# RazorClient/Stark-prover

Measured on AMD Instinct MI355X. Metric: FRI commit field-elems/sec at codeword 2^24; achieved HBM GB/s vs peak, higher is better.
Workload: dtype u32; 1 GPU; fri_commit codeword 2^24, blowup 8 (d=2^21), SHA-256 Merkle per layer, 21 rounds; codeword_log2=24, per_gpu_log2=24, blowup=8, field=p=3*2^30+1, parallelism=single GPU

## Files before the change

stark-prover_amd/csrc/fri_layer.hip:

```cpp
#include <cassert>
#include "fri_internal.hpp"
#include "sha256_fast.hpp"
#include "sha256_quad.hpp"

namespace fri {

#ifdef FRI_STAMPS
#define STAMP_WITH(on, i, fn)                                  \
    do {                                                       \
        if (on) t.st->stamps[t.k][(i)] = fn();                 \
    } while (0)
#else
#define STAMP_WITH(on, i, fn) do {} while (0)
#endif
#define STAMP(on, i) STAMP_WITH(on, i, __builtin_amdgcn_s_memrealtime)
#define STAMP_CLK(on, i) STAMP_WITH(on, i, __builtin_amdgcn_s_memtime)

#ifndef FRI_CHAIN_PRIO
#define FRI_CHAIN_PRIO 3
#endif
__device__ __forceinline__ void chain_prio() {
    if (FRI_CHAIN_PRIO > 0) __builtin_amdgcn_s_setprio(FRI_CHAIN_PRIO);
}

// ... 9 lines not shown
}
__device__ __forceinline__ void dg_lds_load(const uint4* p, Dg& d) {
    uint4 a = p[0], b = p[1];
    d.w[0] = a.x; d.w[1] = a.y; d.w[2] = a.z; d.w[3] = a.w; d.w[4] = b.x; d.w[5] = b.y; d.w[6] = b.z; d.w[7] = b.w;
}
__device__ __forceinline__ void dg_lds_store(uint4* p, const Dg& d) {
    p[0] = make_uint4(d.w[0], d.w[1], d.w[2], d.w[3]);
    p[1] = make_uint4(d.w[4], d.w[5], d.w[6], d.w[7]);
}
__device__ __forceinline__ void hnode(const Dg& l, const Dg& r, Dg& o) { shaf::node(l.w, r.w, o.w); }
__device__ __forceinline__ void hleaf(uint32_t v, Dg& o) { shaf::leaf(v, o.w); }
__device__ __forceinline__ void cnode(const Dg& l, const Dg& r, Dg& o) { shaf::node_compact(l.w, r.w, o.w); }
__device__ __forceinline__ void cleaf(uint32_t v, Dg& o) { shaf::leaf_compact(v, o.w); }

__device__ __forceinline__ void pair_level(const uint4* A, uint4* B, uint32_t* out, uint32_t tid, uint32_t cnt,
                                           const shaq::Role& R) {
    if (tid >= max(2 * cnt, 64u)) return;
    const uint32_t q = (tid >> 1) & (cnt - 1), half = (tid & 1u) ^ 1u;
    const bool real = tid < 2 * cnt;
    Dg a, b;
    dg_lds_load(A + 4 * q, a);
    dg_lds_load(A + 4 * q + 2, b);
    uint32_t o[4];
    shaq::node(a.w, b.w, o, R);
    if (!real) return;
    const uint4 v = make_uint4(o[0], o[1], o[2], o[3]);
    B[2 * q + half] = v;
    reinterpret_cast<uint4*>(out + 8 * q)[half] = v;
}

#ifndef FRI_SCHED_PRODUCER
#define FRI_SCHED_PRODUCER 1
#endif
struct SchedLds {
    uint32_t wk[32 * 48];
    uint32_t flag;
};
__device__ __forceinline__ void sched_init(SchedLds* sl) {
    if (FRI_SCHED_PRODUCER && threadIdx.x == 0) sl->flag = 0u;
}
__device__ __forceinline__ void pair_level_s(const uint4* A, uint4* B, uint32_t* out, uint32_t tid, uint32_t cnt,
                                             const shaq::Role& R, SchedLds* sl, uint32_t ord) {
    if (!FRI_SCHED_PRODUCER || cnt > 32) {
        pair_level(A, B, out, tid, cnt, R);
        return;
    }
    const uint32_t wv = tid >> 6;
    if (wv > 1) return;
    const uint32_t lane = tid & 63u;
    const uint32_t q = (lane >> 1) & (cnt - 1), half = (lane & 1u) ^ 1u;
    const bool real = lane < 2 * cnt;
    Dg a, b;
    dg_lds_load(A + 4 * q, a);
    dg_lds_load(A + 4 * q + 2, b);
    if (wv == 1) {
        uint32_t w[16];
#pragma unroll
        for (int i = 0; i < 8; i++) { w[i] = a.w[i]; w[8 + i] = b.w[i]; }
        shaq::produce(w, sl->wk + 48 * q, &sl->flag, 3u * ord, real && (lane & 1u) == 0u, lane == 0u, R);
        return;
    }
    uint32_t o[4];
    shaq::node_ext(a.w, b.w, o, R, sl->wk + 48 * q, &sl->flag, 3u * ord);
    if (!real) return;
    const uint4 v = make_uint4(o[0], o[1], o[2], o[3]);
    B[2 * q + half] = v;
    reinterpret_cast<uint4*>(out + 8 * q)[half] = v;
}

__device__ __forceinline__ void lds_barrier() {
    asm volatile("s_waitcnt lgkmcnt(0)\n\ts_barrier" ::: "memory");
}

__device__ __forceinline__ int wave_max_i(int v) {
#pragma unroll
    for (int off = 32; off > 0; off >>= 1) v = max(v, __shfl_xor(v, off));
    return v;
}

struct Mx3 {
    int m0 = -1, m1 = -1, m2 = -1;
    __device__ __forceinline__ void load(const int32_t* p, uint32_t i) { m0 = p[3 * i]; m1 = p[3 * i + 1]; m2 = p[3 * i + 2]; }
    __device__ __forceinline__ void take(const int32_t* p, uint32_t i) {
        m0 = max(m0, p[3 * i]); m1 = max(m1, p[3 * i + 1]); m2 = max(m2, p[3 * i + 2]);
    }
    __device__ __forceinline__ void store(int32_t* p, uint32_t i) const { p[3 * i] = m0; p[3 * i + 1] = m1; p[3 * i + 2] = m2; }
    __device__ __forceinline__ void wave_max() { m0 = wave_max_i(m0); m1 = wave_max_i(m1); m2 = wave_max_i(m2); }
};
__device__ __forceinline__ void mx3_wave_to_red(Mx3 m, int32_t* red, uint32_t tx) {
    m.wave_max();
    if ((tx & 63) == 0) m.store(red, tx >> 6);
}
__device__ __forceinline__ Mx3 mx3_from_red(const int32_t* red, uint32_t nw) {
    Mx3 m;
    for (uint32_t i = 0; i < nw; i++) m.take(red, i);
    return m;
}
struct Degree { int deg; bool noncanon; };
__device__ __forceinline__ Degree degree_of(int k, const Mx3& m) {
    return {k == 0 ? m.m0 : (m.m1 < 0 ? m.m2 : m.m0), k == 0 && m.m1 >= 0};
}

__device__ __forceinline__ void coef_slice(const LayerTask& t, uint32_t w, uint32_t G, int32_t* red, uint32_t t0,
                                           uint32_t nthr) {
    Mx3 m;
// ... 83 lines not shown

template <bool FOLD, bool COMMIT, uint32_t TPB, bool PAIR = false>
__global__ __launch_bounds__(TPB) void k_layer_leaf(LayerTask t) {
    if (gated_off(t)) return;
    __shared__ uint4 lds[3 * TPB];
    __shared__ int32_t red[3 * (TPB / 64)];
    const uint32_t L = t.L;
    const size_t wg = PAIR ? (size_t)blockIdx.x + t.wg_base : (size_t)blockIdx.x;
    const size_t q = wg * TPB + threadIdx.x;
    uint4 v;
    if (FOLD) {
        const size_t half = (size_t)1 << L;
        const uint32_t beta_m = COMMIT ? t.st->beta_mont[t.k - 1] : (PAIR ? pair_beta(t) : t.beta_m);
        uint4 a = reinterpret_cast<const uint4*>(t.prev)[q];
        uint4 b = reinterpret_cast<const uint4*>(PAIR ? t.prev2 : t.prev + half)[q];
        uint4 x = reinterpret_cast<const uint4*>(t.xinv)[q];
        v.x = fold_one(a.x, b.x, x.x, beta_m); v.y = fold_one(a.y, b.y, x.y, beta_m);
        v.z = fold_one(a.z, b.z, x.z, beta_m); v.w = fold_one(a.w, b.w, x.w, beta_m);
        reinterpret_cast<uint4*>(t.values)[q] = v;
    } else {
        v = reinterpret_cast<const uint4*>(t.values)[q];
    }
    uint32_t* tr = t.tree;
    Dg top;
    quad(v, tr + 8 * level_offset(L, 0), tr + 8 * level_offset(L, 1), q, top);
    if (COMMIT) coef_task(t, blockIdx.x, gridDim.x, red);
    lds_two_levels<TPB>(lds, top, tr + 8 * level_offset(L, 2), tr + 8 * level_offset(L, 3),
                        tr + 8 * level_offset(L, 4), wg * TPB);
}

#ifndef WIDE_PAIR_MAX
#define WIDE_PAIR_MAX (1u << 16)
#endif

__host__ __device__ __forceinline__ uint32_t wide_levels(uint32_t L) { return L <= 8 + TOP_LOG ? 8u : 4u; }

template <bool FOLD, bool COMMIT, bool PAIR = false>
__global__ __launch_bounds__(256) void k_layer_leaf_wide(LayerTask t) {
    if (gated_off(t)) return;
    STAMP(COMMIT && blockIdx.x == 0 && threadIdx.x == 0, 60);
    __shared__ uint4 lds[2 * 256 + 2 * 128];
    __shared__ int32_t red[12];
    __shared__ SchedLds sl;
    sched_init(&sl);
    const uint32_t L = t.L;
    const size_t wg = PAIR ? (size_t)blockIdx.x + t.wg_base : (size_t)blockIdx.x;
    const size_t grid = PAIR ? (size_t)t.wg_total : (size_t)gridDim.x;
    const size_t i = wg * 256 + threadIdx.x;
    uint32_t v;
    if (FOLD) {
        const size_t half = (size_t)1 << L;
        const uint32_t beta_m = COMMIT ? t.st->beta_mont[t.k - 1] : (PAIR ? pair_beta(t) : t.beta_m);
        v = fold_one(t.prev[i], PAIR ? t.prev2[i] : t.prev[i + half], t.xinv[i], beta_m);
        t.values[i] = v;
    } else {
        v = t.values[i];
    }
    uint32_t* tr = t.tree;
    Dg d;
    cleaf(v, d);
    dg_store(tr + 8 * i, d);
    uint4* A = lds;
    uint4* B = lds + 2 * 256;
    dg_lds_store(A + 2 * threadIdx.x, d);
    lds_barrier();
    STAMP(COMMIT && blockIdx.x == 0 && threadIdx.x == 0, 61);
    uint32_t cnt = 256;
    const shaq::Role qr = shaq::role_of(threadIdx.x);
    if (grid * 128 < WIDE_PAIR_MAX) chain_prio();
    const uint32_t nlev = wide_levels(L);
#pragma unroll 1
    for (uint32_t j = 1; j <= nlev; j++) {
        cnt >>= 1;
        uint32_t* out = tr + 8 * (level_offset(L, j) + (wg << (8 - j)));
        if ((size_t)cnt * grid < WIDE_PAIR_MAX) {
            pair_level_s(A, B, out, threadIdx.x, cnt, qr, &sl, j);
        } else if (threadIdx.x < cnt) {
            Dg a, b, o;
            dg_lds_load(A + 4 * threadIdx.x, a);
            dg_lds_load(A + 4 * threadIdx.x + 2, b);
            hnode(a, b, o);
            dg_lds_store(B + 2 * threadIdx.x, o);
            dg_store(out + 8 * threadIdx.x, o);
        }
        if (COMMIT && j == 2 && threadIdx.x >= 128) coef_slice(t, blockIdx.x, gridDim.x, red, 128, 128);
        lds_barrier();
        uint4* tmp = A; A = B; B = tmp;
    }
    if (COMMIT && threadIdx.x == 128) coef_combine(t, blockIdx.x, red, 2);
    STAMP(COMMIT && blockIdx.x == 0 && threadIdx.x == 0, 62);
}

__device__ __forceinline__ void reduce_mx(const int32_t* in, int32_t* out, uint32_t w, uint32_t R) {
    if (threadIdx.x >= 64) return;
    Mx3 m;
    if (threadIdx.x < R) m.load(in, R * w + threadIdx.x);
    m.wave_max();
    if (threadIdx.x == 0) m.store(out, w);
}

__global__ __launch_bounds__(512) void k_tree_mid(uint32_t* tree, uint32_t L, uint32_t l, const DevState* st,
                                                  int gate, const int32_t* mx_in, int32_t* mx_out, uint32_t R) {
    if (st && gate >= 0 && !st->active[gate]) return;
    constexpr uint32_t NIN = 1024;
    __shared__ uint4 lds[NIN + NIN / 2];
    __shared__ SchedLds sl;
    sched_init(&sl);
    uint4* A = lds;
    uint4* B = lds + NIN;
    const uint32_t t = threadIdx.x;
    const size_t base = (size_t)blockIdx.x * NIN;
    const uint32_t* in = tree + 8 * level_offset(L, l);
    {
        Dg a, b, o;
        dg_load(in + 8 * (base + 2 * t), a);
        dg_load(in + 8 * (base + 2 * t + 1), b);
        if (mx_in) reduce_mx(mx_in, mx_out, blockIdx.x, R);
        hnode(a, b, o);
        dg_lds_store(A + 2 * t, o);
        dg_store(tree + 8 * (level_offset(L, l + 1) + (base >> 1) + t), o);
    }
    lds_barrier();
    const shaq::Role qr = shaq::role_of(t);
    uint32_t cnt = NIN / 2;
#pragma unroll 1
    for (uint32_t j = 2; j <= 4; j++) {
        cnt >>= 1;
        uint32_t* out = tree + 8 * (level_offset(L, l + j) + (base >> j));
        const bool narrow = (size_t)cnt * gridDim.x < WIDE_PAIR_MAX;
        if (narrow) {
            pair_level_s(A, B, out, t, cnt, qr, &sl, j);
        } else if (t < cnt) {
            Dg a, b, o;
            dg_lds_load(A + 4 * t, a);
            dg_lds_load(A + 4 * t + 2, b);
            hnode(a, b, o);
            dg_lds_store(B + 2 * t, o);
            dg_store(out + 8 * t, o);
        }
        lds_barrier();
        uint4* tmp = A; A = B; B = tmp;
    }
}

__global__ __launch_bounds__(256) void k_tree_mid8(uint32_t* tree, uint32_t L, uint32_t l, const DevState* st,
                                                   int gate, const int32_t* mx_in, int32_t* mx_out, uint32_t R) {
    if (st && gate >= 0 && !st->active[gate]) return;
    chain_prio();
    __shared__ uint4 lds[256 + 128];
    __shared__ SchedLds sl;
    sched_init(&sl);
    uint4* A = lds;
    uint4* B = lds + 256;
    const uint32_t t = threadIdx.x;
    const size_t base = (size_t)blockIdx.x * 256;
    const uint32_t* in = tree + 8 * level_offset(L, l);
    const shaq::Role qr = shaq::role_of(t);
    {
        const uint32_t q = t >> 1, half = (t & 1u) ^ 1u;
        Dg a, b;
        dg_load(in + 8 * (base + 2 * q), a);
        dg_load(in + 8 * (base + 2 * q + 1), b);
        if (mx_in) reduce_mx(mx_in, mx_out, blockIdx.x, R);
        uint32_t o[4];
        shaq::node(a.w, b.w, o, qr);
        const uint4 v = make_uint4(o[0], o[1], o[2], o[3]);
        A[2 * q + half] = v;
        reinterpret_cast<uint4*>(tree + 8 * (level_offset(L, l + 1) + (base >> 1) + q))[half] = v;
    }
    lds_barrier();
    uint32_t cnt = 128;
#pragma unroll 1
    for (uint32_t j = 2; j <= 8; j++) {
        cnt >>= 1;
        pair_level_s(A, B, tree + 8 * (level_offset(L, l + j) + (base >> j)), t, cnt, qr, &sl, j);
        lds_barrier();
        uint4* tmp = A; A = B; B = tmp;
    }
}

__device__ __forceinline__ void ktouch(const void* sym) {
    uint32_t a, b, c, d;
    asm volatile("s_nop 4\n\t"
                 "s_load_dword %0, %4, 0x0\n\ts_load_dword %1, %4, 0x40\n\t"
                 "s_load_dword %2, %4, 0x80\n\ts_load_dword %3, %4, 0xc0\n\t"
                 "s_waitcnt lgkmcnt(0)"
                 : "=&s"(a), "=&s"(b), "=&s"(c), "=&s"(d)
                 : "s"(sym)
                 : "memory");
}
__device__ __forceinline__ void kcache_touch_sha_tables() {
    ktouch(&shaf::KTAB[0]);
    ktouch(&shaf::PAD_KW_C.kw[0]);
    ktouch(&shaf::PAD_KW_1024.kw[0]);
    ktouch(&shaf::PAD_KW_1536.kw[0]);
}

__device__ __forceinline__ uint32_t hexch(uint32_t nib) { return nib < 10u ? 0x30u + nib : 0x57u + nib; }
__device__ __forceinline__ void hex2(uint32_t x, uint32_t& hi, uint32_t& lo) {
    hi = (hexch(x >> 28) << 24) | (hexch((x >> 24) & 15u) << 16) | (hexch((x >> 20) & 15u) << 8) | hexch((x >> 16) & 15u);
    lo = (hexch((x >> 12) & 15u) << 24) | (hexch((x >> 8) & 15u) << 16) | (hexch((x >> 4) & 15u) << 8) | hexch(x & 15u);
}
__device__ __forceinline__ uint32_t hexhex(uint32_t b) {
    const uint32_t x = ((b & 0xF0u) << 12) | (b & 0x0Fu);
    const uint32_t ge = ((x + 0x00060006u) >> 4) & 0x00010001u;
    return 0x33303330u + x + ge * 0x2F7u;
}

enum { CJ_REHASH = 0, CJ_MID = 2, CJ_ROOT = 3, CJ_FINAL = 6, CJ_END_ROUND = 6, CJ_END_FINAL = 8 };

__device__ __forceinline__ void chan_job(int j, uint32_t cs[8], uint32_t X[4], uint32_t has, const uint4* root_lds,
// ... 65 lines not shown
            dg_lds_store(A + 2 * j, d);
        }
    }
}

__device__ __forceinline__ void level_step(const LayerTask& t, bool stamps, uint32_t it, const uint4* A, uint4* B,
                                           uint32_t* out, uint32_t cnt, const shaq::Role& R, SchedLds* sl,
                                           uint32_t ord) {
    const uint32_t tid = threadIdx.x;
    if (cnt <= 128) {
        STAMP_CLK(stamps && it < 18 && tid == 0, 24 + 2 * it);
        pair_level_s(A, B, out, tid, cnt, R, sl, ord);
        STAMP_CLK(stamps && it < 18 && tid == 0, 25 + 2 * it);
        return;
    }
#pragma unroll 1
    for (uint32_t q = tid; q < cnt; q += blockDim.x) {
        Dg a, b, o;
        dg_lds_load(A + 4 * q, a);
        dg_lds_load(A + 4 * q + 2, b);
#ifdef FRI_STAMPS
        if (stamps && it < 18 && q == 0) asm volatile("s_waitcnt lgkmcnt(0)" ::: "memory");
#endif
        STAMP_CLK(stamps && it < 18 && q == 0, 24 + 2 * it);
        cnode(a, b, o);
        STAMP_CLK(stamps && it < 18 && q == 0, 25 + 2 * it);
        dg_lds_store(B + 2 * q, o);
        dg_store(out + 8 * q, o);
    }
}

__device__ __forceinline__ int chan_drain(const LayerTask& t, int job, int job_end, bool level, uint32_t cnt,
                                           uint32_t cs[8], uint32_t X[4], uint32_t has, const uint4* root_lds,
                                           uint32_t fv, const shaq::Role& R) {
    if (job >= job_end || (level && !(cnt <= 192 && job < CJ_ROOT))) return job;
    do {
        STAMP(threadIdx.x == 448 && job == CJ_ROOT, 14);
        STAMP(threadIdx.x == 448 && job == CJ_ROOT + 2, 13);
        chan_job(job, cs, X, has, root_lds, fv, R);
        STAMP(threadIdx.x == 448 && job >= CJ_ROOT && job <= CJ_ROOT + 2, 20 + job - CJ_ROOT);
        job++;
    } while (!level && job < job_end);
    return job;
}

struct RoundOut { uint32_t active, beta_m; };
__device__ __forceinline__ RoundOut layer_results(const LayerTask& t, const Degree& dg, const uint32_t cs[8],
                                                  uint32_t fv, uint32_t fbeta1, const uint4* root_lds) {
    DevState* st = t.st;
    const int k = t.k, deg = dg.deg;
    if (dg.noncanon) {
        st->active[k] = 0;
        st->status = 1u;
        return {0u, 0u};
    }
    st->deg[k] = deg;
    Dg root;
    dg_lds_load(root_lds, root);
#pragma unroll
    for (int i = 0; i < 8; i++) st->roots[k][i] = root.w[i];
    st->n_layers = (uint32_t)k + 1;
    STAMP(true, 15);
    if (deg >= 1 && k < MAXR && t.L >= 1) {
        uint32_t beta = chan_beta(cs);
#pragma unroll
        for (int i = 0; i < 8; i++) st->chan[i] = cs[i];
        st->chan_has = 1;
        st->chan_pending = 1;
        if (fbeta1) beta = fbeta1 - 1u;
        st->beta[k] = beta;
        const uint32_t bm = to_mont(beta);
        st->beta_mont[k] = bm;
        st->active[k] = 1;
        st->n_rounds = (uint32_t)k + 1;
        STAMP(true, 16);
        return {1u, bm};
    }
    st->active[k] = 0;
    if (deg >= 1) { st->status = 7u; return {0u, 0u}; }
#pragma unroll
    for (int i = 0; i < 8; i++) st->chan[i] = cs[i];
    st->final_value = fv;
    st->final_degree = deg;
    st->chan_has = 1;
    st->chan_pending = 0;
    return {0u, 0u};
}

template <bool FROM_LEAVES, bool COMMIT, bool SHARD = false>
__global__ __launch_bounds__(512) void k_tree_top(LayerTask t, uint32_t l, const int32_t* mx, uint32_t G) {
    static_assert(!(FROM_LEAVES && (COMMIT || SHARD)), "from the leaves: standalone trees only");
    if (gated_off(t)) return;
    chain_prio();
    __shared__ uint4 lds[2 * 1024 + 2 * 512];
    __shared__ int32_t red[24];
    __shared__ SchedLds sl;
    sched_init(&sl);
    const uint32_t L = t.L;
    const uint32_t N = 1u << (L - l);
    const uint32_t tid = threadIdx.x;

    const bool chan_wave = COMMIT && tid >= 448;
    DevState* st = t.st;
    uint32_t cs[8], X[4];
    uint32_t has = 0, fbeta1 = 0;
    int job = CJ_END_FINAL;
    if (chan_wave) {
#pragma unroll
        for (int i = 0; i < 8; i++) cs[i] = st->chan[i];
        const uint32_t h = st->chan_has, pend = st->chan_pending;
        const uint32_t fo = COMMIT ? st->forced : 0u, fb = st->forced_beta[t.k < MAXR ? t.k : 0];
        has = h;
        job = !h ? CJ_ROOT : (pend ? CJ_REHASH : CJ_MID);
        if (fo && t.k < MAXR) fbeta1 = fb + 1u;
    }
    if (tid >= 384 && tid < 448) kcache_touch_sha_tables();
    uint4* A = lds;
    uint4* B = lds + 2 * 1024;
    uint32_t* tr = t.tree;
    STAMP(COMMIT && tid == 0, 0);
    if (FROM_LEAVES) {
        leaf_loop(N, tr, A, [&](uint32_t j, bool) { return t.values[j]; });
    } else if (SHARD && COMMIT) {
        const ShardTop& sh = *t.shard;
        for (uint32_t i = tid; i < N; i += blockDim.x) {
            Dg d;
            dg_load(sh.recs_in + REC_WORDS * sh.rank_of_block[i], d);
            dg_lds_store(A + 2 * i, d);
            dg_store(tr + 8 * i, d);
        }
// ... 2 lines not shown
            m.load(reinterpret_cast<const int32_t*>(sh.recs_in + REC_WORDS * tid + 8), 0);
            if (sh.sched_on) { m.m0 = sh.sched_deg; m.m1 = t.k == 0 ? -1 : 0; m.m2 = -1; }
        }
        mx3_wave_to_red(m, red, tid);
    } else {
        const uint32_t* in = tr + 8 * level_offset(L, l);
        Mx3 m;
        if (COMMIT && tid < G) m.load(mx, tid);
        for (uint32_t i = tid; i < N; i += blockDim.x) {
            Dg d;
            dg_load(in + 8 * i, d);
            dg_lds_store(A + 2 * i, d);
        }
        if (SHARD && !COMMIT) {
            const ShardTop& sh = *t.shard;
            for (uint32_t i = tid; i < sh.rec_R; i += blockDim.x) m.take(sh.rec_mx, i);
            mx3_wave_to_red(m, red, tid);
        }
        if (COMMIT) {
            for (uint32_t i = tid + blockDim.x; i < G; i += blockDim.x) m.take(mx, i);
            mx3_wave_to_red(m, red, tid);
        }
    }
    lds_barrier();
    const Degree dg = COMMIT ? degree_of(t.k, mx3_from_red(red, 8)) : Degree{-1, false};
    const bool is_final = COMMIT && dg.deg < 1;
    const int job_end = is_final ? CJ_END_FINAL : CJ_END_ROUND;
    uint32_t fv = 0;
    if (chan_wave && is_final && dg.deg == 0)
        fv = SHARD ? t.shard->recs_in[11] : (t.k == 0 ? t.coef_in : t.coef_out)[0];
    STAMP(COMMIT && tid == 0, 1);
    STAMP_CLK(COMMIT && tid == 0, 17);
    const uint32_t nlev = L - l;
    const uint32_t total = nlev + (COMMIT ? 1u : 0u);
    const shaq::Role R = shaq::role_of(tid);
    uint32_t cnt = N;
#pragma unroll 1
    for (uint32_t it = 0; it < total; it++) {
        const bool level = it < nlev;
        if (level) {
            cnt >>= 1;
            level_step(t, COMMIT, it, A, B, tr + 8 * level_offset(L, l + 1 + it), cnt, R, &sl, it);
        }
        if (chan_wave) job = chan_drain(t, job, job_end, level, cnt, cs, X, has, A, fv, R);
        lds_barrier();
        if (level) {
            uint4* tmp = A; A = B; B = tmp;
            STAMP(COMMIT && tid == 0 && it < 11, 2 + it);
            STAMP_CLK(COMMIT && tid == 0 && it + 1 == nlev, 18);
            STAMP(COMMIT && tid == 0 && it + 1 == nlev, 19);
        }
    }
    if (SHARD && !COMMIT && tid == 448) {
        const ShardTop& sh = *t.shard;
        const Mx3 m = mx3_from_red(red, 8);
        Dg root;
        dg_lds_load(A, root);
        uint32_t* rec = sh.rec_out;
        dg_store(rec, root);
        reinterpret_cast<uint4*>(rec)[2] = make_uint4((uint32_t)m.m0, (uint32_t)m.m1, (uint32_t)m.m2, sh.rec_c0[0]);
        reinterpret_cast<uint4*>(rec)[3] = make_uint4(0u, 0u, 0u, 0u);
    }
    if (COMMIT && tid == 448) layer_results(t, dg, cs, fv, fbeta1, A);
}

struct TailTask {
    LayerTask t[TAIL_LOG + 1];
    uint32_t n;
};

template <bool FOLD0>
__global__ __launch_bounds__(512) void k_tree_tail(TailTask tt) {
    const LayerTask& t0 = tt.t[0];
    if (gated_off(t0)) return;
    chain_prio();
    constexpr uint32_t NMAX = 1u << TAIL_LOG;
    __shared__ uint4 lds[2 * NMAX + NMAX];
    __shared__ uint32_t vals[2][NMAX];
    __shared__ uint32_t coefs[2][NMAX];
    __shared__ int32_t red[24];
    __shared__ uint32_t s_beta_m, s_active;
    __shared__ int32_t s_deg;
    __shared__ uint32_t s_fbeta[TAIL_LOG + 2];
    __shared__ uint32_t xv[2 * NMAX];
    __shared__ SchedLds sl;
    sched_init(&sl);
    uint32_t ord = 0;
    const uint32_t tid = threadIdx.x;
    const bool chan_wave = tid >= 448;
    DevState* st = t0.st;
    auto prefetch_x = [&](uint32_t t0p, uint32_t nthr) {
        uint32_t off = 1u << tt.t[0].L;
        for (uint32_t li = 1; li < tt.n; li++) {
            const uint32_t N = 1u << tt.t[li].L;
            for (uint32_t j = tid - t0p; j < N; j += nthr) xv[off + j] = tt.t[li].xinv[j];
            off += N;
        }
    };
    uint32_t cs[8], X[4];
    uint32_t has = 0;
    if (chan_wave) {
#pragma unroll
        for (int i = 0; i < 8; i++) cs[i] = st->chan[i];
        has = st->chan_has;
    }
    uint32_t pending = chan_wave ? st->chan_pending : 0u;
    if (tid >= 384 && tid < 448) kcache_touch_sha_tables();
    if (tid < tt.n + 1) {
        const int kk = t0.k + (int)tid;
        s_fbeta[tid] = (st->forced && kk < MAXR) ? st->forced_beta[kk] + 1u : 0u;
    }
    uint32_t beta_m = FOLD0 ? st->beta_mont[t0.k - 1] : 0u;
    int prev_deg = FOLD0 ? st->deg[t0.k - 1] : -1;
    const shaq::Role R = shaq::role_of(tid);
    uint32_t xoff = 0;
#pragma unroll 1
    for (uint32_t li = 0; li < tt.n; li++) {
        const LayerTask& t = tt.t[li];
        const int k = t.k;
        const uint32_t L = t.L, N = 1u << L;
        const uint32_t* xl = li ? xv + xoff : t.xinv;
        xoff += N;
        const bool fold = FOLD0 || li > 0;
        uint32_t* cur_v = vals[li & 1];
        const uint32_t* prev_v = vals[(li & 1) ^ 1];
        uint32_t* cur_c = coefs[li & 1];
        const uint32_t* prev_c = coefs[(li & 1) ^ 1];
        uint4* A = lds;
        uint4* B = lds + 2 * NMAX;
        uint32_t* tr = t.tree;
        STAMP(tid == 0, 0);
        leaf_loop(N, tr, A, [&](uint32_t j, bool real) {
            uint32_t v;
            if (fold) {
                const uint32_t a = li ? prev_v[j] : t.prev[j], b = li ? prev_v[j + N] : t.prev[j + N];
                v = fold_one(a, b, xl[j], beta_m);
                if (real) t.values[j] = v;
            } else {
                v = t.values[j];
            }
            if (real) cur_v[j] = v;
            return v;
        });
        const uint32_t nlev = L;
        const uint32_t coef_it = N > 256 ? 1u : 0u;
        const bool coef_late = nlev > coef_it;
        auto coef_fold = [&](uint32_t t0c, uint32_t nthr) {
            Mx3 m;
            const uint32_t tx = tid - t0c;
            if (k == 0) {
                for (size_t j = tx; j < t.d0; j += nthr) {
                    const uint32_t c = t.coef_in[j];
                    if (c) m.m0 = max(m.m0, (int)j);
                    if (c >= P) m.m1 = 0;
                }
            } else {
                const uint32_t len = (uint32_t)(prev_deg + 1), nlen = (len + 1) / 2;
                const bool in_lds = li > 0 && k >= 2;
                for (uint32_t j = tx; j < nlen; j += nthr) {
                    const uint32_t e = in_lds ? prev_c[2 * j] : t.coef_in[2 * j];
                    const uint32_t o = (2 * j + 1 < len) ? (in_lds ? prev_c[2 * j + 1] : t.coef_in[2 * j + 1]) : 0u;
                    const uint32_t v = add(e, mmul(o, beta_m));
                    cur_c[j] = v;
                    if (v) m.m0 = (int)j;
                    if (e) m.m1 = (int)j;
                    if (o) m.m2 = (int)j;
                }
            }
            mx3_wave_to_red(m, red, tx);
        };
        if (!coef_late) coef_fold(0, blockDim.x);
        if (li == 0 && !coef_late) prefetch_x(0, blockDim.x);
        lds_barrier();
        STAMP(tid == 0, 1);
        STAMP_CLK(tid == 0, 17);
        Degree dg{1, false};
        int job_end = CJ_END_ROUND;
        uint32_t fv = 0;
        auto settle = [&](uint32_t nw) {
            dg = degree_of(k, mx3_from_red(red, nw));
            job_end = dg.deg < 1 ? CJ_END_FINAL : CJ_END_ROUND;
            if (chan_wave && dg.deg == 0) fv = (k == 0) ? t.coef_in[0] : cur_c[0];
        };
        if (!coef_late) settle(8);
        int job = CJ_END_FINAL;
        if (chan_wave) job = !has ? CJ_ROOT : (pending ? CJ_REHASH : CJ_MID);
        const uint32_t total = nlev + 1;
        uint32_t cnt = N;
#pragma unroll 1
        for (uint32_t it = 0; it < total; it++) {
            const bool level = it < nlev;
            if (level) {
                cnt >>= 1;
                level_step(t, true, it, A, B, tr + 8 * level_offset(L, 1 + it), cnt, R, &sl, ord++);
            }
            if (chan_wave) job = chan_drain(t, job, job_end, level, cnt, cs, X, has, A, fv, R);
            if (coef_late && it == coef_it && tid >= 256 && tid < 384) coef_fold(256, 128);
            if (li == 0 && coef_late && it == coef_it && tid >= 384 && tid < 448) prefetch_x(384, 64);
            lds_barrier();
            if (coef_late && it == coef_it) settle(2);
            if (level) {
                uint4* tmp = A; A = B; B = tmp;
                STAMP(tid == 0 && it < 11, 2 + it);
                STAMP_CLK(tid == 0 && it + 1 == nlev, 18);
                STAMP(tid == 0 && it + 1 == nlev, 19);
            }
        }
        if (tid == 448) {
            const RoundOut r = layer_results(t, dg, cs, fv, s_fbeta[li], A);
            s_beta_m = r.beta_m;
            s_active = r.active;
            s_deg = dg.deg;
        }
        if (chan_wave) { has = 1; pending = 1; }
        lds_barrier();
        if (!s_active) break;
        beta_m = s_beta_m;
        prev_deg = s_deg;
    }
}

__global__ __launch_bounds__(512) void k_commit_batch(BatchTask bt) {
    constexpr uint32_t NMAX = 1u << TAIL_LOG;
    __shared__ uint4 lds[2 * NMAX + NMAX];
    __shared__ uint32_t vals[2][NMAX];
    __shared__ uint32_t coefs[2][NMAX];
    __shared__ int32_t red[24];
    __shared__ uint32_t s_beta_m, s_active;
    __shared__ int32_t s_deg;
    __shared__ uint32_t s_fbeta[BATCH_MAX_LOG + 2];
    __shared__ SchedLds sl;
    sched_init(&sl);
    uint32_t ord = 0;
    const uint32_t tid = threadIdx.x;
    const bool chan_wave = tid >= 448;
    const size_t mb = blockIdx.x;
    DevState* st = bt.st + mb;
    uint32_t* layers = bt.layers + mb * bt.lay_stride;
    uint32_t* trees = bt.trees + mb * bt.tre_stride;
    const uint32_t* input = bt.coef_in + mb * bt.in_stride;
    uint32_t* cA = bt.coefA + mb * bt.coef_stride;
    uint32_t* cB = bt.coefB + mb * bt.coef_stride;
    auto cbuf = [&](int r) -> uint32_t* { return (r & 1) ? cA : cB; };
    uint32_t cs[8], X[4];
    uint32_t has = 0;
    if (chan_wave) {
#pragma unroll
        for (int i = 0; i < 8; i++) cs[i] = st->chan[i];
        has = st->chan_has;
    }
    uint32_t pending = chan_wave ? st->chan_pending : 0u;
    if (tid >= 384 && tid < 448) kcache_touch_sha_tables();
    if (tid < (uint32_t)bt.rmax + 2)
        s_fbeta[tid] = (st->forced && tid < (uint32_t)MAXR) ? st->forced_beta[tid] + 1u : 0u;
    uint32_t beta_m = 0u;
    int prev_deg = -1;
    const shaq::Role R = shaq::role_of(tid);
#pragma unroll 1
    for (int k = 0; k <= bt.rmax; k++) {
        const uint32_t L = bt.log_n - (uint32_t)k, N = 1u << L;
        LayerTask t{};
        t.st = st;
        t.k = k;
        t.L = L;
        const bool big = L > TAIL_LOG;
// ... 23 lines not shown
                uint32_t* cout = big ? cbuf(k) : cur_c;
                for (uint32_t j = tid; j < nlen; j += blockDim.x) {
                    const uint32_t e = cin[2 * j];
                    const uint32_t o = (2 * j + 1 < len) ? cin[2 * j + 1] : 0u;
                    const uint32_t v = add(e, mmul(o, beta_m));
                    cout[j] = v;
                    if (v) m.m0 = (int)j;
                    if (e) m.m1 = (int)j;
                    if (o) m.m2 = (int)j;
                }
            }
            mx3_wave_to_red(m, red, tid);
        }
        uint32_t N2 = N, lvl0 = 0;
        if (big) {
            const uint32_t tiles = N >> TAIL_LOG;
#pragma unroll 1
            for (uint32_t tile = 0; tile < tiles; tile++) {
                A = lds;
                B = lds + 2 * NMAX;
                const uint32_t i = (tile << TAIL_LOG) + tid;
                uint32_t v;
                if (k) {
                    v = fold_one(prev[i], prev[i + N], xl[i], beta_m);
                    values[i] = v;
                } else {
                    v = values[i];
                }
                Dg d;
                cleaf(v, d);
                dg_store(tr + 8 * (size_t)i, d);
                dg_lds_store(A + 2 * tid, d);
                lds_barrier();
                uint32_t cnt = NMAX;
#pragma unroll 1
                for (uint32_t j = 1; j <= TAIL_LOG; j++) {
                    cnt >>= 1;
                    level_step(t, false, 0, A, B, tr + 8 * (level_offset(L, j) + ((size_t)tile << (TAIL_LOG - j))), cnt,
                               R, &sl, ord++);
                    lds_barrier();
                    uint4* tmp = A; A = B; B = tmp;
                }
            }
            __syncthreads();
            N2 = tiles;
            lvl0 = TAIL_LOG;
            A = lds;
            B = lds + 2 * NMAX;
            const uint32_t* in = tr + 8 * level_offset(L, TAIL_LOG);
            for (uint32_t i = tid; i < N2; i += blockDim.x) {
                Dg d;
                dg_load(in + 8 * i, d);
                dg_lds_store(A + 2 * i, d);
            }
        } else {
            leaf_loop(N, tr, A, [&](uint32_t j, bool real) {
                uint32_t v;
                if (k) {
                    const uint32_t a = prev_lds ? prev_v[j] : prev[j], b = prev_lds ? prev_v[j + N] : prev[j + N];
                    v = fold_one(a, b, xl[j], beta_m);
                    if (real) values[j] = v;
                } else {
                    v = values[j];
                }
                if (real) cur_v[j] = v;
                return v;
            });
        }
        lds_barrier();
        const Degree dg = degree_of(k, mx3_from_red(red, 8));
        const int job_end = dg.deg < 1 ? CJ_END_FINAL : CJ_END_ROUND;
        uint32_t fv = 0;
        if (chan_wave && dg.deg == 0) fv = (k == 0) ? input[0] : (big ? cbuf(k)[0] : cur_c[0]);
        int job = CJ_END_FINAL;
        if (chan_wave) job = !has ? CJ_ROOT : (pending ? CJ_REHASH : CJ_MID);
        const uint32_t nlev = L - lvl0;
        const uint32_t total = nlev + 1;
        uint32_t cnt = N2;
#pragma unroll 1
        for (uint32_t it = 0; it < total; it++) {
            const bool level = it < nlev;
            if (level) {
                cnt >>= 1;
                level_step(t, false, it, A, B, tr + 8 * level_offset(L, lvl0 + 1 + it), cnt, R, &sl, ord++);
            }
            if (chan_wave) job = chan_drain(t, job, job_end, level, cnt, cs, X, has, A, fv, R);
            lds_barrier();
            if (level) {
                uint4* tmp = A; A = B; B = tmp;
            }
        }
        if (tid == 448) {
            const RoundOut r = layer_results(t, dg, cs, fv, s_fbeta[k], A);
            s_beta_m = r.beta_m;
            s_active = r.active;
            s_deg = dg.deg;
        }
        if (chan_wave) { has = 1; pending = 1; }
        __syncthreads();
        if (!s_active) break;
        beta_m = s_beta_m;
        prev_deg = s_deg;
    }
}

void launch_commit_batch(const BatchTask& bt, uint32_t batch, hipStream_t s) {
    assert(bt.log_n >= 1 && bt.log_n <= BATCH_MAX_LOG && bt.rmax <= (int)bt.log_n);
    hipLaunchKernelGGL(k_commit_batch, dim3(batch), dim3(512), 0, s, bt);
}

__global__ __launch_bounds__(256) void k_batch_scale(const uint32_t* __restrict__ src, size_t src_stride,
                                                     uint32_t* __restrict__ dst, size_t dst_stride, size_t d,
                                                     const uint32_t* __restrict__ lo, const uint32_t* __restrict__ hi) {
    const size_t j = (size_t)blockIdx.x * 256 + threadIdx.x;
    if (j >= d) return;
    const uint32_t v = src[blockIdx.y * src_stride + j];
    dst[blockIdx.y * dst_stride + j] = mmul(mmul(v, hi[j >> POW_LO_LOG]), lo[j & ((1u << POW_LO_LOG) - 1)]);
}
void launch_batch_scale(const uint32_t* src, size_t src_stride, uint32_t* dst, size_t dst_stride, size_t d,
                        uint32_t batch, const uint32_t* lo, const uint32_t* hi, hipStream_t s) {
    if (!d) return;
    hipLaunchKernelGGL(k_batch_scale, dim3((unsigned)((d + 255) / 256), batch), dim3(256), 0, s, src, src_stride, dst,
                       dst_stride, d, lo, hi);
}

__global__ __launch_bounds__(256) void k_batch_lde_lds(const uint32_t* __restrict__ src, size_t src_stride, uint32_t d,
// ... 10 lines not shown
        a[__brev(j) >> (32 - log_n)] = v;
    }
    __syncthreads();
#pragma unroll 1
    for (uint32_t s = 0; s < log_n; s++) {
        const uint32_t half = 1u << s;
        for (uint32_t idx = threadIdx.x; idx < n / 2; idx += 256) {
            const uint32_t j = idx & (half - 1), p0 = ((idx >> s) << (s + 1)) + j;
            const uint32_t u = a[p0], w = mmul(a[p0 + half], tw[half + j]);
            a[p0] = add(u, w);
            a[p0 + half] = sub(u, w);
        }
        __syncthreads();
    }
    for (uint32_t j = threadIdx.x; j < n; j += 256) out[j] = a[j];
}
void launch_batch_lde_lds(const uint32_t* src, size_t src_stride, size_t d, uint32_t* layers, size_t lay_stride,
                          uint32_t log_n, uint32_t batch, const uint32_t* tw, const uint32_t* lo, const uint32_t* hi,
                          hipStream_t s) {
    assert(log_n >= 1 && log_n <= BATCH_LDS_LDE_MAX_LOG && d <= ((size_t)1 << log_n));
    hipLaunchKernelGGL(k_batch_lde_lds, dim3(batch), dim3(256), 0, s, src, src_stride, (uint32_t)d, layers, lay_stride,
                       log_n, tw, lo, hi);
}

static LayerTask with_gate(const LayerTask& in) {
    LayerTask t = in;
    if (t.st) { t.gst = t.st; t.gidx = t.k > 0 ? t.k - 1 : -1; }
    return t;
}

#ifndef QUAD_TPB
#define QUAD_TPB 512
#endif
#ifndef QUAD_MIN_LOG
#define QUAD_MIN_LOG 19
#endif

template <typename KernelLaunch>
static void pair_parts(LayerTask t, uint32_t G, hipStream_t s, const std::function<void()>& after_part1,
                       KernelLaunch&& go) {
    t.wg_total = G;
    if (!after_part1) {
        t.wg_base = 0;
        go(t, G);
        return;
    }
    const uint32_t h = G / 2;
    t.wg_base = t.send_half ? h : 0u;
    go(t, h);
    after_part1();
    t.wg_base = t.send_half ? 0u : h;
    go(t, h);
}

void launch_layer(const LayerTask& tin, hipStream_t s, hipEvent_t ev_leaf_end, const std::function<void()>& after_leaf,
                  hipEvent_t ev_before_top, const std::function<void()>& after_part1) {
    const LayerTask t = with_gate(tin);
    const uint32_t L = t.L;
    const bool fold = t.prev != nullptr;
    const bool commit = t.st != nullptr;
    const bool pair = t.prev2 != nullptr;
    const int32_t* nomx = nullptr;
    static_assert(TAIL_LOG == TOP_LOG, "every commit layer the top could take from its leaves goes to launch_tail");
    if (L <= TOP_LOG) {
        assert(!fold && !commit);
        hipLaunchKernelGGL((k_tree_top<true, false>), dim3(1), dim3(512), 0, s, t, 0u, nomx, 1u);
        if (ev_leaf_end) hipEventRecord(ev_leaf_end, s);
        return;
    }
    uint32_t G, out_per_wg;
// ... 87 lines not shown
```

Before: 3.648 billion field-elems/s.

## Run narrow Merkle levels barrier-free with wave-specialized producer/consumer phase

Adds a narrow phase for Merkle levels with at most 32 nodes. Instead of a workgroup barrier per level, wave 0 computes the SHA nodes and keeps intermediates in registers, wave 1 produces message schedules, and wave 2 writes nodes to global memory. The waves hand off through an LDS level counter using acquire/release spins. The channel drain now waits on that counter for the root instead of interleaving with each level, and the tail kernel schedules its coefficient fold earlier. This targets barrier latency on the serial top-of-tree levels, at the cost of spin-waits, extra LDS, and more complex synchronization.

```diff
diff --git a/stark-prover_amd/csrc/fri_layer.hip b/stark-prover_amd/csrc/fri_layer.hip
--- a/stark-prover_amd/csrc/fri_layer.hip
+++ b/stark-prover_amd/csrc/fri_layer.hip
@@ -65,6 +65,12 @@
 #ifndef FRI_SCHED_PRODUCER
 #define FRI_SCHED_PRODUCER 1
 #endif
+#ifndef FRI_NARROW_PHASE
+#define FRI_NARROW_PHASE 1
+#endif
+#if FRI_NARROW_PHASE && !FRI_SCHED_PRODUCER
+#error "the narrow phase runs its nodes through the schedule producer"
+#endif
 struct SchedLds {
     uint32_t wk[32 * 48];
     uint32_t flag;
@@ -74,7 +80,7 @@
 }
 __device__ __forceinline__ void pair_level_s(const uint4* A, uint4* B, uint32_t* out, uint32_t tid, uint32_t cnt,
                                              const shaq::Role& R, SchedLds* sl, uint32_t ord) {
-    if (!FRI_SCHED_PRODUCER || cnt > 32) {
+    if (!FRI_SCHED_PRODUCER || FRI_NARROW_PHASE || cnt > 32) {
         pair_level(A, B, out, tid, cnt, R);
         return;
     }
@@ -104,6 +110,92 @@
 __device__ __forceinline__ void lds_barrier() {
     asm volatile("s_waitcnt lgkmcnt(0)\n\ts_barrier" ::: "memory");
 }
+
+constexpr uint32_t NARROW_MAX = 32;
+struct NarrowLds {
+    uint4 nd[128];
+    uint32_t lvl;
+};
+__device__ __forceinline__ void narrow_init(NarrowLds* nl) {
+    if (FRI_NARROW_PHASE && threadIdx.x == 0) nl->lvl = 0u;
+}
+__device__ __forceinline__ uint4* narrow_at(NarrowLds* nl, uint32_t cnt) { return nl->nd + (128u - 4u * cnt); }
+__device__ __forceinline__ void lvl_wait(const uint32_t* lvl, uint32_t v) {
+    while (__hip_atomic_load(lvl, __ATOMIC_ACQUIRE, __HIP_MEMORY_SCOPE_WORKGROUP) < v) {}
+}
+__device__ __forceinline__ void lvl_wait_idle(const uint32_t* lvl, uint32_t v) {
+    while (__hip_atomic_load(lvl, __ATOMIC_ACQUIRE, __HIP_MEMORY_SCOPE_WORKGROUP) < v) __builtin_amdgcn_s_sleep(2);
+}
+struct NarrowStamps { const LayerTask* stp; uint32_t node0, done0, nmax; };
+#ifdef FRI_STAMPS
+#define NSTAMP(on, i, fn)                                                      \
+    do {                                                                       \
+        if (ns.stp && lane == 0 && (on)) ns.stp->st->stamps[ns.stp->k][(i)] = fn(); \
+    } while (0)
+#else
+#define NSTAMP(on, i, fn) do {} while (0)
+#endif
+template <typename Chan>
+__device__ __forceinline__ const uint4* narrow_phase(const uint4* A, uint32_t cnt, uint32_t n, uint32_t* tree,
+                                                     uint32_t L, uint32_t j0, size_t base0, const shaq::Role& R,
+                                                     SchedLds* sl, NarrowLds* nl, uint32_t ord0,
+                                                     const NarrowStamps& ns, Chan&& chan) {
+    const uint32_t wv = threadIdx.x >> 6, lane = threadIdx.x & 63u;
+    const uint4* last = n ? narrow_at(nl, cnt >> (n - 1)) : A;
+    if (wv == 0) {
+        const uint32_t half = (lane & 1u) ^ 1u;
+        Dg a, b;
+        if (n) {
+            const uint32_t q = (lane >> 1) & (cnt - 1);
+            dg_lds_load(A + 4 * q, a);
+            dg_lds_load(A + 4 * q + 2, b);
+        }
+#pragma unroll 1
+        for (uint32_t i = 0; i < n; i++, cnt >>= 1) {
+            const uint32_t q = (lane >> 1) & (cnt - 1);
+            NSTAMP(i < ns.nmax, ns.node0 + 2 * i, __builtin_amdgcn_s_memtime);
+            uint32_t o[4];
+            shaq::node_ext(a.w, b.w, o, R, sl->wk + 48 * q, &sl->flag, 3u * (ord0 + i));
+            NSTAMP(i < ns.nmax, ns.node0 + 2 * i + 1, __builtin_amdgcn_s_memtime);
+            uint4* dst = narrow_at(nl, cnt);
+            if (lane < 2 * cnt) dst[2 * q + half] = make_uint4(o[0], o[1], o[2], o[3]);
+            if (i + 1 < n) {
+                const uint32_t qn = (lane >> 1) & ((cnt >> 1) - 1);
+                dg_lds_load(dst + 4 * qn, a);
+                dg_lds_load(dst + 4 * qn + 2, b);
+            }
+            if (lane == 0) __hip_atomic_store(&nl->lvl, ord0 + i + 1, __ATOMIC_RELEASE, __HIP_MEMORY_SCOPE_WORKGROUP);
+            NSTAMP(ns.done0 && i < ns.nmax, ns.done0 + i, __builtin_amdgcn_s_memrealtime);
+        }
+    } else if (wv == 1) {
+        const uint4* src = A;
+#pragma unroll 1
+        for (uint32_t i = 0; i < n; i++, cnt >>= 1) {
+            if (i) lvl_wait(&nl->lvl, ord0 + i);
+            const uint32_t q = (lane >> 1) & (cnt - 1);
+            Dg a, b;
+            dg_lds_load(src + 4 * q, a);
+            dg_lds_load(src + 4 * q + 2, b);
+            uint32_t w[16];
+#pragma unroll
+            for (int x = 0; x < 8; x++) { w[x] = a.w[x]; w[8 + x] = b.w[x]; }
+            shaq::produce(w, sl->wk + 48 * q, &sl->flag, 3u * (ord0 + i), lane < 2 * cnt && (lane & 1u) == 0u,
+                          lane == 0u, R);
+            src = narrow_at(nl, cnt);
+        }
+    } else if (wv == 2) {
+#pragma unroll 1
+        for (uint32_t i = 0; i < n; i++, cnt >>= 1) {
+            lvl_wait_idle(&nl->lvl, ord0 + i + 1);
+            uint4* out = reinterpret_cast<uint4*>(tree + 8 * (level_offset(L, j0 + i) + (base0 >> (j0 + i))));
+            if (lane < 2 * cnt) out[lane] = narrow_at(nl, cnt)[lane];
+        }
+    } else {
+        chan(last, n ? ord0 + n : 0u);
+    }
+    return last;
+}
+#undef NSTAMP
 
 __device__ __forceinline__ int wave_max_i(int v) {
 #pragma unroll
@@ -253,6 +345,9 @@
 #ifndef WIDE_PAIR_MAX
 #define WIDE_PAIR_MAX (1u << 16)
 #endif
+#ifndef QUAD_MIN_LOG
+#define QUAD_MIN_LOG 19
+#endif
 
 __host__ __device__ __forceinline__ uint32_t wide_levels(uint32_t L) { return L <= 8 + TOP_LOG ? 8u : 4u; }
 
@@ -263,7 +358,9 @@
     __shared__ uint4 lds[2 * 256 + 2 * 128];
     __shared__ int32_t red[12];
     __shared__ SchedLds sl;
+    __shared__ NarrowLds nl;
     sched_init(&sl);
+    narrow_init(&nl);
     const uint32_t L = t.L;
     const size_t wg = PAIR ? (size_t)blockIdx.x + t.wg_base : (size_t)blockIdx.x;
     const size_t grid = PAIR ? (size_t)t.wg_total : (size_t)gridDim.x;
@@ -290,8 +387,10 @@
     const shaq::Role qr = shaq::role_of(threadIdx.x);
     if (grid * 128 < WIDE_PAIR_MAX) chain_prio();
     const uint32_t nlev = wide_levels(L);
-#pragma unroll 1
-    for (uint32_t j = 1; j <= nlev; j++) {
+    static_assert(NARROW_MAX << (QUAD_MIN_LOG - 1 - 8) < WIDE_PAIR_MAX, "narrow levels run on lane pairs");
+    const uint32_t nbar = FRI_NARROW_PHASE ? 2u : nlev;
+#pragma unroll 1
+    for (uint32_t j = 1; j <= nbar; j++) {
         cnt >>= 1;
         uint32_t* out = tr + 8 * (level_offset(L, j) + (wg << (8 - j)));
         if ((size_t)cnt * grid < WIDE_PAIR_MAX) {
@@ -307,6 +406,11 @@
         if (COMMIT && j == 2 && threadIdx.x >= 128) coef_slice(t, blockIdx.x, gridDim.x, red, 128, 128);
         lds_barrier();
         uint4* tmp = A; A = B; B = tmp;
+    }
+    if (FRI_NARROW_PHASE) {
+        const NarrowStamps ns{COMMIT && blockIdx.x == 0 ? &t : nullptr, 42u, 0u, 6u};
+        narrow_phase(A, cnt >> 1, nlev - nbar, tr, L, nbar + 1, wg * 256, qr, &sl, &nl, nbar + 1, ns,
+                     [](const uint4*, uint32_t) {});
     }
     if (COMMIT && threadIdx.x == 128) coef_combine(t, blockIdx.x, red, 2);
     STAMP(COMMIT && blockIdx.x == 0 && threadIdx.x == 0, 62);
@@ -370,7 +474,9 @@
     chain_prio();
     __shared__ uint4 lds[256 + 128];
     __shared__ SchedLds sl;
+    __shared__ NarrowLds nl;
     sched_init(&sl);
+    narrow_init(&nl);
     uint4* A = lds;
     uint4* B = lds + 256;
     const uint32_t t = threadIdx.x;
@@ -391,13 +497,17 @@
     }
     lds_barrier();
     uint32_t cnt = 128;
-#pragma unroll 1
-    for (uint32_t j = 2; j <= 8; j++) {
+    const uint32_t nbar = FRI_NARROW_PHASE ? 2u : 8u;
+#pragma unroll 1
+    for (uint32_t j = 2; j <= nbar; j++) {
         cnt >>= 1;
         pair_level_s(A, B, tree + 8 * (level_offset(L, l + j) + (base >> j)), t, cnt, qr, &sl, j);
         lds_barrier();
         uint4* tmp = A; A = B; B = tmp;
     }
+    if (FRI_NARROW_PHASE)
+        narrow_phase(A, cnt >> 1, 8 - nbar, tree, L, l + nbar + 1, base << l, qr, &sl, &nl, nbar + 1,
+                     NarrowStamps{nullptr, 0u, 0u, 0u}, [](const uint4*, uint32_t) {});
 }
 
 __device__ __forceinline__ void ktouch(const void* sym) {
@@ -529,9 +639,14 @@
 
 __device__ __forceinline__ int chan_drain(const LayerTask& t, int job, int job_end, bool level, uint32_t cnt,
                                            uint32_t cs[8], uint32_t X[4], uint32_t has, const uint4* root_lds,
-                                           uint32_t fv, const shaq::Role& R) {
+                                           uint32_t fv, const shaq::Role& R, const uint32_t* lvl, uint32_t root_lvl) {
     if (job >= job_end || (level && !(cnt <= 192 && job < CJ_ROOT))) return job;
+    bool rooted = !FRI_NARROW_PHASE || root_lvl == 0u;
     do {
+        if (!rooted && job >= CJ_ROOT) {
+            lvl_wait(lvl, root_lvl);
+            rooted = true;
+        }
         STAMP(threadIdx.x == 448 && job == CJ_ROOT, 14);
         STAMP(threadIdx.x == 448 && job == CJ_ROOT + 2, 13);
         chan_job(job, cs, X, has, root_lds, fv, R);
@@ -592,7 +707,9 @@
     __shared__ uint4 lds[2 * 1024 + 2 * 512];
     __shared__ int32_t red[24];
     __shared__ SchedLds sl;
+    __shared__ NarrowLds nl;
     sched_init(&sl);
+    narrow_init(&nl);
     const uint32_t L = t.L;
     const uint32_t N = 1u << (L - l);
     const uint32_t tid = threadIdx.x;
@@ -661,36 +778,38 @@
     STAMP(COMMIT && tid == 0, 1);
     STAMP_CLK(COMMIT && tid == 0, 17);
     const uint32_t nlev = L - l;
-    const uint32_t total = nlev + (COMMIT ? 1u : 0u);
     const shaq::Role R = shaq::role_of(tid);
-    uint32_t cnt = N;
-#pragma unroll 1
-    for (uint32_t it = 0; it < total; it++) {
-        const bool level = it < nlev;
-        if (level) {
-            cnt >>= 1;
-            level_step(t, COMMIT, it, A, B, tr + 8 * level_offset(L, l + 1 + it), cnt, R, &sl, it);
-        }
-        if (chan_wave) job = chan_drain(t, job, job_end, level, cnt, cs, X, has, A, fv, R);
+    uint32_t cnt = N, it = 0;
+#pragma unroll 1
+    for (; it < nlev && (!FRI_NARROW_PHASE || (cnt >> 1) > NARROW_MAX); it++) {
+        cnt >>= 1;
+        level_step(t, COMMIT, it, A, B, tr + 8 * level_offset(L, l + 1 + it), cnt, R, &sl, it);
+        if (!FRI_NARROW_PHASE && chan_wave)
+            job = chan_drain(t, job, job_end, true, cnt, cs, X, has, A, fv, R, &nl.lvl, 0u);
         lds_barrier();
-        if (level) {
-            uint4* tmp = A; A = B; B = tmp;
-            STAMP(COMMIT && tid == 0 && it < 11, 2 + it);
-            STAMP_CLK(COMMIT && tid == 0 && it + 1 == nlev, 18);
-            STAMP(COMMIT && tid == 0 && it + 1 == nlev, 19);
-        }
-    }
+        uint4* tmp = A; A = B; B = tmp;
+        STAMP(COMMIT && tid == 0 && it < 11, 2 + it);
+    }
+    const uint4* root = narrow_phase(
+        A, cnt >> 1, nlev - it, tr, L, l + 1 + it, 0, R, &sl, &nl, it,
+        NarrowStamps{COMMIT ? &t : nullptr, 24u + 2u * it, 2u + it, 9u - it},
+        [&](const uint4* root_lds, uint32_t root_lvl) {
+            if (chan_wave) job = chan_drain(t, job, job_end, false, 0u, cs, X, has, root_lds, fv, R, &nl.lvl, root_lvl);
+        });
+    STAMP_CLK(COMMIT && tid == 0, 18);
+    STAMP(COMMIT && tid == 0, 19);
+    lds_barrier();
     if (SHARD && !COMMIT && tid == 448) {
         const ShardTop& sh = *t.shard;
         const Mx3 m = mx3_from_red(red, 8);
-        Dg root;
-        dg_lds_load(A, root);
+        Dg root_dg;
+        dg_lds_load(root, root_dg);
         uint32_t* rec = sh.rec_out;
-        dg_store(rec, root);
+        dg_store(rec, root_dg);
         reinterpret_cast<uint4*>(rec)[2] = make_uint4((uint32_t)m.m0, (uint32_t)m.m1, (uint32_t)m.m2, sh.rec_c0[0]);
         reinterpret_cast<uint4*>(rec)[3] = make_uint4(0u, 0u, 0u, 0u);
     }
-    if (COMMIT && tid == 448) layer_results(t, dg, cs, fv, fbeta1, A);
+    if (COMMIT && tid == 448) layer_results(t, dg, cs, fv, fbeta1, root);
 }
 
 struct TailTask {
@@ -713,7 +832,9 @@
     __shared__ uint32_t s_fbeta[TAIL_LOG + 2];
     __shared__ uint32_t xv[2 * NMAX];
     __shared__ SchedLds sl;
+    __shared__ NarrowLds nl;
     sched_init(&sl);
+    narrow_init(&nl);
     uint32_t ord = 0;
     const uint32_t tid = threadIdx.x;
     const bool chan_wave = tid >= 448;
@@ -773,7 +894,8 @@
         });
         const uint32_t nlev = L;
         const uint32_t coef_it = N > 256 ? 1u : 0u;
-        const bool coef_late = nlev > coef_it;
+        const bool coef_early = FRI_NARROW_PHASE && nlev > 0 && N <= 2 * NARROW_MAX;
+        const bool coef_late = !coef_early && nlev > coef_it;
         auto coef_fold = [&](uint32_t t0c, uint32_t nthr) {
             Mx3 m;
             const uint32_t tx = tid - t0c;
@@ -798,8 +920,13 @@
             }
             mx3_wave_to_red(m, red, tx);
         };
-        if (!coef_late) coef_fold(0, blockDim.x);
-        if (li == 0 && !coef_late) prefetch_x(0, blockDim.x);
+        if (coef_early) {
+            if (tid >= 256 && tid < 384) coef_fold(256, 128);
+            if (li == 0 && tid >= 384 && tid < 448) prefetch_x(384, 64);
+        } else if (!coef_late) {
+            coef_fold(0, blockDim.x);
+            if (li == 0) prefetch_x(0, blockDim.x);
+        }
         lds_barrier();
         STAMP(tid == 0, 1);
         STAMP_CLK(tid == 0, 17);
@@ -811,32 +938,38 @@
             job_end = dg.deg < 1 ? CJ_END_FINAL : CJ_END_ROUND;
             if (chan_wave && dg.deg == 0) fv = (k == 0) ? t.coef_in[0] : cur_c[0];
         };
-        if (!coef_late) settle(8);
+        if (coef_early) settle(2);
+        else if (!coef_late) settle(8);
         int job = CJ_END_FINAL;
         if (chan_wave) job = !has ? CJ_ROOT : (pending ? CJ_REHASH : CJ_MID);
-        const uint32_t total = nlev + 1;
-        uint32_t cnt = N;
-#pragma unroll 1
-        for (uint32_t it = 0; it < total; it++) {
-            const bool level = it < nlev;
-            if (level) {
-                cnt >>= 1;
-                level_step(t, true, it, A, B, tr + 8 * level_offset(L, 1 + it), cnt, R, &sl, ord++);
-            }
-            if (chan_wave) job = chan_drain(t, job, job_end, level, cnt, cs, X, has, A, fv, R);
+        uint32_t cnt = N, it = 0;
+#pragma unroll 1
+        for (; it < nlev && (!FRI_NARROW_PHASE || (cnt >> 1) > NARROW_MAX); it++) {
+            cnt >>= 1;
+            level_step(t, true, it, A, B, tr + 8 * level_offset(L, 1 + it), cnt, R, &sl, ord++);
+            if (!FRI_NARROW_PHASE && chan_wave)
+                job = chan_drain(t, job, job_end, true, cnt, cs, X, has, A, fv, R, &nl.lvl, 0u);
             if (coef_late && it == coef_it && tid >= 256 && tid < 384) coef_fold(256, 128);
             if (li == 0 && coef_late && it == coef_it && tid >= 384 && tid < 448) prefetch_x(384, 64);
             lds_barrier();
             if (coef_late && it == coef_it) settle(2);
-            if (level) {
-                uint4* tmp = A; A = B; B = tmp;
-                STAMP(tid == 0 && it < 11, 2 + it);
-                STAMP_CLK(tid == 0 && it + 1 == nlev, 18);
-                STAMP(tid == 0 && it + 1 == nlev, 19);
-            }
-        }
+            uint4* tmp = A; A = B; B = tmp;
+            STAMP(tid == 0 && it < 11, 2 + it);
+        }
+        const uint32_t nn = nlev - it;
+        const uint4* root = narrow_phase(
+            A, cnt >> 1, nn, tr, L, 1 + it, 0, R, &sl, &nl, ord,
+            NarrowStamps{&t, 24u + 2u * it, 2u + it, 9u - it},
+            [&](const uint4* root_lds, uint32_t root_lvl) {
+                if (chan_wave)
+                    job = chan_drain(t, job, job_end, false, 0u, cs, X, has, root_lds, fv, R, &nl.lvl, root_lvl);
+            });
+        ord += nn;
+        STAMP_CLK(tid == 0, 18);
+        STAMP(tid == 0, 19);
+        lds_barrier();
         if (tid == 448) {
-            const RoundOut r = layer_results(t, dg, cs, fv, s_fbeta[li], A);
+            const RoundOut r = layer_results(t, dg, cs, fv, s_fbeta[li], root);
             s_beta_m = r.beta_m;
             s_active = r.active;
             s_deg = dg.deg;
@@ -859,7 +992,9 @@
     __shared__ int32_t s_deg;
     __shared__ uint32_t s_fbeta[BATCH_MAX_LOG + 2];
     __shared__ SchedLds sl;
+    __shared__ NarrowLds nl;
     sched_init(&sl);
+    narrow_init(&nl);
     uint32_t ord = 0;
     const uint32_t tid = threadIdx.x;
     const bool chan_wave = tid >= 448;
@@ -949,14 +1084,21 @@
                 dg_store(tr + 8 * (size_t)i, d);
                 dg_lds_store(A + 2 * tid, d);
                 lds_barrier();
-                uint32_t cnt = NMAX;
-#pragma unroll 1
-                for (uint32_t j = 1; j <= TAIL_LOG; j++) {
+                uint32_t cnt = NMAX, j = 1;
+#pragma unroll 1
+                for (; j <= TAIL_LOG && (!FRI_NARROW_PHASE || (cnt >> 1) > NARROW_MAX); j++) {
                     cnt >>= 1;
                     level_step(t, false, 0, A, B, tr + 8 * (level_offset(L, j) + ((size_t)tile << (TAIL_LOG - j))), cnt,
                                R, &sl, ord++);
                     lds_barrier();
                     uint4* tmp = A; A = B; B = tmp;
+                }
+                if (FRI_NARROW_PHASE) {
+                    const uint32_t nn = TAIL_LOG + 1 - j;
+                    narrow_phase(A, cnt >> 1, nn, tr, L, j, (size_t)tile << TAIL_LOG, R, &sl, &nl, ord,
+                                 NarrowStamps{nullptr, 0u, 0u, 0u}, [](const uint4*, uint32_t) {});
+                    ord += nn;
+                    lds_barrier();
                 }
             }
             __syncthreads();
@@ -992,23 +1134,27 @@
         int job = CJ_END_FINAL;
         if (chan_wave) job = !has ? CJ_ROOT : (pending ? CJ_REHASH : CJ_MID);
         const uint32_t nlev = L - lvl0;
-        const uint32_t total = nlev + 1;
-        uint32_t cnt = N2;
-#pragma unroll 1
-        for (uint32_t it = 0; it < total; it++) {
-            const bool level = it < nlev;
-            if (level) {
-                cnt >>= 1;
-                level_step(t, false, it, A, B, tr + 8 * level_offset(L, lvl0 + 1 + it), cnt, R, &sl, ord++);
-            }
-            if (chan_wave) job = chan_drain(t, job, job_end, level, cnt, cs, X, has, A, fv, R);
+        uint32_t cnt = N2, it = 0;
+#pragma unroll 1
+        for (; it < nlev && (!FRI_NARROW_PHASE || (cnt >> 1) > NARROW_MAX); it++) {
+            cnt >>= 1;
+            level_step(t, false, it, A, B, tr + 8 * level_offset(L, lvl0 + 1 + it), cnt, R, &sl, ord++);
+            if (!FRI_NARROW_PHASE && chan_wave)
+                job = chan_drain(t, job, job_end, true, cnt, cs, X, has, A, fv, R, &nl.lvl, 0u);
             lds_barrier();
-            if (level) {
-                uint4* tmp = A; A = B; B = tmp;
-            }
-        }
+            uint4* tmp = A; A = B; B = tmp;
+        }
+        const uint32_t nn = nlev - it;
+        const uint4* root = narrow_phase(
+            A, cnt >> 1, nn, tr, L, lvl0 + 1 + it, 0, R, &sl, &nl, ord, NarrowStamps{nullptr, 0u, 0u, 0u},
+            [&](const uint4* root_lds, uint32_t root_lvl) {
+                if (chan_wave)
+                    job = chan_drain(t, job, job_end, false, 0u, cs, X, has, root_lds, fv, R, &nl.lvl, root_lvl);
+            });
+        ord += nn;
+        lds_barrier();
         if (tid == 448) {
-            const RoundOut r = layer_results(t, dg, cs, fv, s_fbeta[k], A);
+            const RoundOut r = layer_results(t, dg, cs, fv, s_fbeta[k], root);
             s_beta_m = r.beta_m;
             s_active = r.active;
             s_deg = dg.deg;
@@ -1085,10 +1231,6 @@
 #ifndef QUAD_TPB
 #define QUAD_TPB 512
 #endif
-#ifndef QUAD_MIN_LOG
-#define QUAD_MIN_LOG 19
-#endif
-
 template <typename KernelLaunch>
 static void pair_parts(LayerTask t, uint32_t G, hipStream_t s, const std::function<void()>& after_part1,
                        KernelLaunch&& go) {
```

After: 3.631 billion field-elems/s. Within noise of the previous version (-0.5%).
